# utiasSTARS/pyslam

Hardware: AMD Instinct MI355X
Metric: ms/LM-iter (Jac build + J^T J + Schur solve), stereo BA @ 500k residuals (lower is better)
Workload: dtype f64

## Files before the change

pyslam_amd/csrc/ps_abi_problem.h:

```cpp


const char* ps_last_error(void) { return g_err.c_str(); }

int ps_device_count(void) {
    int n = 0;
    if (hipGetDeviceCount(&n) != hipSuccess) return 0;
    return n;
}

int ps_warm_up(void) {
    static std::once_flag once;
    static int rc = 0;
    std::call_once(once, [] {
        void* p = nullptr;
        if (hipMalloc(&p, 256) != hipSuccess) { rc = fail("hipMalloc failed (no usable HIP device?)"); return; }
        hipLaunchKernelGGL(k_zero4, dim3(1), dim3(256), 0, 0, (size_t)8, (double*)p, (size_t)0, (double*)nullptr, (size_t)0,
                           (double*)nullptr, (size_t)0, (double*)nullptr);
        double hostw[4] = {0, 0, 0, 0};
        (void)hipMemsetAsync(p, 0, 256, 0);
        (void)hipMemcpyAsync((char*)p + 128, p, 64, hipMemcpyDeviceToDevice, 0);
        (void)hipMemcpyAsync(hostw, p, sizeof(hostw), hipMemcpyDeviceToHost, 0);
        if (hipDeviceSynchronize() != hipSuccess) rc = fail("the warm-up launch failed");
        hipFree(p);
        hipFuncAttributes a;
#define PS_TOUCH(...) (void)hipFuncGetAttributes(&a, reinterpret_cast<const void*>(&__VA_ARGS__))
        PS_TOUCH(k_landmark_pass<false>); PS_TOUCH(k_landmark_pass_packed<false, false>); PS_TOUCH(k_landmark_pass_packed<false, true>); PS_TOUCH(k_backsub_packed<false>); PS_TOUCH(k_pose_pass<false>); PS_TOUCH(k_pose_finalize); PS_TOUCH(k_schur_pairs_db<0>);
        PS_TOUCH(k_schur_combine); PS_TOUCH(k_backsub<false>); PS_TOUCH(k_cost_reproj<false>); PS_TOUCH(k_cost_packed<false>); PS_TOUCH(k_reduce3); PS_TOUCH(k_reduce_partials);
        PS_TOUCH(k_copy2); PS_TOUCH(k_zero4); PS_TOUCH(k_lag_status_check);
        PS_TOUCH(k_block_jacobi_factor<6>); PS_TOUCH(k_scale_blocks<6>); PS_TOUCH(k_scale_blocks_p<6>); PS_TOUCH(k_rows_setup<6>);
        PS_TOUCH(k_coarse_rowsums<6>); PS_TOUCH(k_coarse_matrix<6>); PS_TOUCH(k_coarse_chol<6, true>); PS_TOUCH(k_coarse_border<6>);
        PS_TOUCH(k_coarse_mreduce<6>); PS_TOUCH(k_coarse_xbuild<6>); PS_TOUCH(k_coarse_recover<6>); PS_TOUCH(k_cg_fused_lds<6, 8>);
        PS_TOUCH(k_cg_fused<6, 8>); PS_TOUCH(k_cg_unscale<6>); PS_TOUCH(k_update_poses<6>); PS_TOUCH(k_update_points);
        PS_TOUCH(k_xcoarse_rowsums<6>); PS_TOUCH(k_xcoarse_matrix<6>); PS_TOUCH(k_band_chol<6>); PS_TOUCH(k_band_inverse); PS_TOUCH(k_band_inverse_rl<false>);
        PS_TOUCH(k_band_inverse_rl<true>); PS_TOUCH(k_bp_v); PS_TOUCH(k_bp_t); PS_TOUCH(k_bp_w); PS_TOUCH(k_bp_dense_sep); PS_TOUCH(k_bp_dense);
        PS_TOUCH(k_xcg_restrict<6>); PS_TOUCH(k_xcg_f2_coarse<6, 3>); PS_TOUCH(k_xcg_fused1<6, 8, false>); PS_TOUCH(k_xcg_fused1<6, 0, true>);
        PS_TOUCH(k_xcg_fused1<6, 2, false>); PS_TOUCH(k_xcg_fused1<6, 6, false>);
        PS_TOUCH(k_factor_pass<6>); PS_TOUCH(k_factor_assemble<6>); PS_TOUCH(k_cost_factors<6>);
        PS_TOUCH(k_factor_pass<3>); PS_TOUCH(k_factor_assemble<3>); PS_TOUCH(k_cost_factors<3>); PS_TOUCH(k_block_jacobi_factor<3>);
        PS_TOUCH(k_update_poses<3>); PS_TOUCH(k_direct_solve<6>); PS_TOUCH(k_direct_solve<3>);
        PS_TOUCH(k_motion_only_solve<false>); PS_TOUCH(k_motion_only_iteration<false>);
        PS_TOUCH(k_pcg_spmv<6>); PS_TOUCH(k_pcg_spmv<3>); PS_TOUCH(k_ldi_init); PS_TOUCH(k_ldi_update); PS_TOUCH(k_ldi_gemm); PS_TOUCH(k_ldi_mirror);
        PS_TOUCH(k_ldi_ritz); PS_TOUCH(k_ldi_seed_prep); PS_TOUCH(k_ldi_fro_total); PS_TOUCH(k_ldi_pad_identity);
        PS_TOUCH(k_ldi_scaled_dense<6>); PS_TOUCH(k_ldi_sym_unscale<6>); PS_TOUCH(k_ldi_scaled_dense<3>); PS_TOUCH(k_ldi_sym_unscale<3>);
        PS_TOUCH(k_shard_pack<6>); PS_TOUCH(k_shard_unpack<6>); PS_TOUCH(k_publish); PS_TOUCH(k_cov_rhs); PS_TOUCH(k_triangulate<false>);
        PS_TOUCH(k_scale_blocks<3>); PS_TOUCH(k_rows_setup<3>); PS_TOUCH(k_coarse_rowsums<3>); PS_TOUCH(k_coarse_matrix<3>);
        PS_TOUCH(k_coarse_chol<3, true>); PS_TOUCH(k_coarse_border<3>); PS_TOUCH(k_coarse_mreduce<3>); PS_TOUCH(k_coarse_xbuild<3>);
        PS_TOUCH(k_coarse_recover<3>); PS_TOUCH(k_cg_fused_lds<3, 8>); PS_TOUCH(k_cg_unscale<3>);
#undef PS_TOUCH
    });
    return rc;
}

int ps_problem_destroy(ps_problem* h) {
    if (!h) return 0;
    if (h->cp_dbg) {
        long long c[8]; hipMemcpy(c, h->cp_dbg, 64, hipMemcpyDeviceToHost);
        int khz = 100000; hipDeviceGetAttribute(&khz, hipDeviceAttributeWallClockRate, 0);
        fprintf(stderr, "k_cg_persist, workgroup 0, %ld launches, us per launch: recurrences %.2f | sync %.2f | products + publish %.2f | gather + sums %.2f "
                "(%.1f failed passes) | dots + sync %.2f | exchanges %lld = %.2f per launch\n", h->cp_launches, c[0] * 1e3 / khz / h->cp_launches,
                c[1] * 1e3 / khz / h->cp_launches, c[2] * 1e3 / khz / h->cp_launches, c[3] * 1e3 / khz / h->cp_launches, (double)c[7] / h->cp_launches,
                c[5] * 1e3 / khz / h->cp_launches, c[6], (double)c[6] / h->cp_launches);
        hipFree(h->cp_dbg);
    }
    if (h->xp_dbg) {
        std::vector<long long> c(3 * 64 * 8); hipMemcpy(c.data(), h->xp_dbg, c.size() * 8, hipMemcpyDeviceToHost);
        int khz = 100000; hipDeviceGetAttribute(&khz, hipDeviceAttributeWallClockRate, 0);
        for (int w = 0; w < 3; ++w) {
            double ph[6] = {0, 0, 0, 0, 0, 0}; int np = 0;
// ... 813 lines not shown
```

pyslam_amd/csrc/ps_abi_solver.h:

```cpp

int ps_get_info(ps_problem* h, ps_problem_info* info) {
    if (!h || !info) return fail("null argument");
    info->dof = h->D; info->num_poses = h->P; info->num_reduced = h->nr; info->num_points = h->L;
    info->num_var_points = h->nv; info->num_obs = h->N; info->num_edges = h->F; info->num_priors = 0;
    info->reduced_nnzb = h->nnzb; info->num_pairs = h->npairs;
    info->reduce_count = ((long)h->nnzb + h->nr) / 2 * h->D * h->D + (long)h->nr * h->D + 3;
    info->device_bytes = (int64_t)h->dev_bytes;
    info->cg_restarts = h->cg_fallbacks;
    info->cg_kernel_launches = h->cg_kernel_launches;
    info->ldi_solves = h->ldi_solves; info->ldi_fallbacks = h->ldi_fallbacks; info->ldi_seeds = h->ldi_seeds;
    info->xcg_fused_solves = h->xf_solves; info->xcg_fused_fallbacks = h->xf_fallbacks;
    info->cg_persist_solves = h->cp_launches; info->cg_persist_failures = h->cp_failures;
    info->cg_persist_refused = h->cp_refused; info->persist_cus = h->persist_cus;
    info->persist_cus_needed = h->cp_ok ? h->cp_cus_needed : (h->xp_ok ? h->xp_cus_needed : 0);
    info->landmark_passes_taken_over = h->prelm_used;
    return 0;
}

int ps_eval_cost(ps_problem* h, int include_all_constant, double* cost) {
    if (!h || !cost) return fail("null argument");
    if (include_all_constant && h->fuse_cost == 1 && lm_cost_possible(h)) { if (lm_cost_pass(h, h->lin_lambda, SC_COST)) return -1; }
    else if (cost_pass(h, include_all_constant, SC_COST)) return -1;
    if (read_scalars(h)) return -1;
    *cost = h->h_scalars[SC_COST];
// ... 794 lines not shown
            for (; i + 8 <= buf.size(); i += 8) { uint64_t w; std::memcpy(&w, &buf[i], 8); hsh = (hsh ^ w) * 1099511628211ull; }
            for (; i < buf.size(); ++i) hsh = (hsh ^ buf[i]) * 1099511628211ull;
        }
        out[t] = hsh;
    }
    return 0;
}

static void relook_path(ps_problem* h) {
    const bool possible = ps_ldi_possible(*h, (long)h->nr * h->D);
    if (h->coarse_built && possible != h->xmin_auto_ldi && h->cg_explicit_min_rows < 0) h->coarse_built = false;
}

int ps_set_option(ps_problem* h, const char* name, double value) {
    if (!h || !name) return fail("null argument");
    if (!std::strcmp(name, "expect_next")) { h->expect_next = value != 0 && !h->hybrid; return 0; }
    if (!std::strcmp(name, "solve_horizon")) { h->solve_horizon = value < 0 ? -1 : (int)std::min(value, 1e6); return 0; }
    if (!std::strcmp(name, "setup_ride")) {
        h->setup_ride = value != 0 ? 1 : 0;
        h->prelin_valid = h->prelm_valid = false;
        relook_launch_gates(h);
        return 0;
    }
    h->prelin_valid = h->prelm_valid = h->ride_valid = false;
    const char* refusal = nullptr;
    const int fx = ps_option_apply(*h, name, value, &refusal);
    if (fx == PS_OPT_UNKNOWN) return fail(std::string("unknown option: ") + name);
    if (fx == PS_OPT_REFUSED) return fail(refusal);
    if (fx & PS_FX_COARSE_REBUILD) h->coarse_built = false;
    if (fx & PS_FX_DROP_FACTOR) h->lci_next = -1;
    if (fx & PS_FX_DROP_SIDE) h->side_todo = false;
    if ((fx & PS_FX_LDI_OFF) && !h->ldi_enable) { h->ldi_cur = -1; if (h->ldi_state != 1) h->ldi_state = 0; }
    if (fx & PS_FX_RELOOK_PATH) relook_path(h);
    relook_launch_gates(h);
    return 0;
}

int ps_get_option(ps_problem* h, const char* name, double* value) {
    if (!h || !name || !value) return fail("null argument");
    const std::string n(name);
    if (n == "lin_zero_list") *value = h->lin_zero_gate ? 1.0 : 0.0;
    else if (n == "lin_fills") *value = (double)h->lin_fills;
    else if (n == "lin_zero_launches") *value = (double)h->lin_zero_launches;
    else if (n == "setup_ride") *value = h->ride_gate ? 1.0 : 0.0;
    else if (n == "factor_launches") *value = (double)h->bjf_launches;
    else if (n == "factors_ridden") *value = (double)h->bjf_ridden;
    else if (n == "factor_plan_mismatches") *value = (double)h->bjf_mismatches;
    else return fail("ps_get_option: no read-back for option: " + n);
    return 0;
}

int ps_reset_solver_state(ps_problem* h) {
    if (!h) return fail("null argument");
    h->prelin_valid = h->prelm_valid = h->ride_valid = false;
    if (!h->solver_touched) {
        static_cast<PsCostHistory&>(*h) = PsCostHistory{};
        return 0;
    }
    h->solver_touched = false;
    HIP_OK(hipStreamSynchronize(h->stream));
    if (h->side) HIP_OK(hipStreamSynchronize(h->side));
    if (h->ldi_stream) HIP_OK(hipStreamSynchronize(h->ldi_stream));
    drain_timers(h);
    static_cast<PsCarried&>(*h) = PsCarried{};
    static_cast<PsCostHistory&>(*h) = PsCostHistory{};
    if (h->lag_status) HIP_OK(hipMemsetAsync(h->lag_status, 0, ST_NWORDS * sizeof(int32_t), h->stream));
    if (h->ldi_ready && !(h->ldi_direct_ok && h->N == 0 && h->F > 0)) h->ldi_direct = false;
    h->cov_ready = false;
    return 0;
}
// ... 54 lines not shown
```

pyslam_amd/csrc/ps_core.hip:

```cpp
#include <hip/hip_runtime.h>

#include <algorithm>
#include <array>
#include <map>
#include <atomic>
#include <chrono>
#include <thread>
#include <climits>
#include <cmath>
#include <cstdio>
#include <cstring>
#include <memory>
#include <mutex>
#include <string>
#include <vector>

#include "pyslam_hip.h"
#include "ps_kernels.h"
#include "ps_ransac.h"
#include "ps_k_twoview.h"
#include "ps_k_pnp.h"
#include "ps_photo.h"
#include "ps_k_dense.h"
#include "ps_k_feat.h"
// ... 207 lines not shown
    long bjf_launches = 0, bjf_ridden = 0, bjf_mismatches = 0;
    std::vector<int32_t> h_row_ptr, h_col_idx;
    std::vector<int32_t> h_vid_of_slot;
    double *x = nullptr, *r = nullptr, *z = nullptr, *p0 = nullptr, *p1 = nullptr, *q = nullptr, *Minv = nullptr;
    double *rz_part = nullptr, *rr_part = nullptr, *pq_part = nullptr, *hist = nullptr;
    int npartA = 0, npartB = 0, hist_cap = 0;
    double *Linv = nullptr, *cg_r[2] = {}, *cg_w[2] = {}, *cg_s[2] = {}, *cg_gd[2] = {}, *cg_xh = nullptr;
    int32_t* brow_of = nullptr;
    double* cg_p = nullptr;
    double* Saug = nullptr;
    int32_t* ident_slot = nullptr;
    int G = 0, ncb = 0, nc = 0, nr_aug = 0, nnzb_aug = 0;
    size_t cg_cap = 0, saug_cap = 0;
    int32_t *pnode = nullptr, *slo = nullptr, *shi = nullptr, *run_lo = nullptr, *run_hi = nullptr,
            *arow_ptr = nullptr, *acol_idx = nullptr, *aug_slot = nullptr, *fine_nnz = nullptr;
    double *pw0 = nullptr, *pw1 = nullptr, *SZ = nullptr, *Ac = nullptr, *tvec = nullptr, *chol_scratch = nullptr;
    double *Bmat = nullptr, *bgv = nullptr, *SB = nullptr, *BSZ = nullptr;
    double *Bmat2[2] = {}, *X2[2] = {}, *Mpart = nullptr;
    bool lagx_ok = false;
    int side_buf = 0;
    double host_wait_ns = 0.0, host_call_ns = 0.0;
    long host_waits = 0, host_calls = 0;
    size_t rows_lds = 0;
    bool rows_attr_set = false, rows_lci_lds = false;
    int32_t *ent_ptr = nullptr, *ent_q = nullptr, *ent_lo = nullptr, *ent_hi = nullptr;
    int32_t *seg_ptr = nullptr, *seg_ent = nullptr, *seg_row = nullptr;
    int max_row_ents = 0;
    int32_t* pose_of_rid = nullptr;
    double *Lci2[2] = {}, *LciT2[2] = {};
    hipStream_t side = nullptr;
    int side_cus = 0;
    hipEvent_t ev_ac = nullptr, ev_chol = nullptr, ev_acdone = nullptr;
    unsigned long long* chk_sums = nullptr; int chk_nsum = 0;
    double *chk_Ac = nullptr, *chk_BSZ = nullptr, *chk_Ac_side = nullptr; int32_t* chk_cnt = nullptr; size_t chk_bsz_n = 0;
    int32_t* lag_status = nullptr;
    double* Mc = nullptr;
    bool coarse_built = false;
    bool coarse_clamped = false;
    int max_pose_obs = 0;
    double* mo_partials = nullptr;
    bool status_clean = true;
    double *dA = nullptr, *dLi = nullptr, *dLiT = nullptr;
    bool cg_explicit = false;
    double lin_lambda = 0.0;
    double *xstate = nullptr, *xy = nullptr, *xp2 = nullptr;
    int ac_bw = -1;
    std::unique_ptr<BandPart> bpart;
// ... 272 lines not shown
```

pyslam_amd/csrc/ps_host_cg.h:

```cpp

namespace {

struct StageTimer {
    ps_problem* h;
    int stage;
    hipEvent_t a = nullptr, b = nullptr;
    int slot = -1;
    StageTimer(ps_problem* h_, int st, int level = 2) : h(h_), stage(st) {
        if (h->profiling < level) return;
        if (h->profiling == 1 && h->prof_every > 1 &&
            h->prof_tick % h->prof_every != (st == PS_ST_CG_KERNEL ? h->prof_every / 2 : 0)) return;
        if (h->ev_used + 2 > h->ev_pool.size()) {
            for (int i = 0; i < 64; ++i) { hipEvent_t e; hipEventCreate(&e); h->ev_pool.push_back(e); }
        }
        slot = (int)h->ev_used;
        a = h->ev_pool[h->ev_used++];
        b = h->ev_pool[h->ev_used++];
        hipEventRecord(a, h->stream);
    }
    void stop() {
        if (!a) return;
        hipEventRecord(b, h->stream);
        h->pending.push_back({stage, slot});
        a = nullptr;
// ... 331 lines not shown
            for (int k = 0; k < nt; ++k) tasks.push_back(CpTask{i, arp[i] + k * per, std::min(arp[i] + w, arp[i] + (k + 1) * per), 0});
        }
        rt0[rows] = (int32_t)tasks.size();
        const int cp_nwg = cdiv((int)tasks.size(), PS_CP_NT / 64);
        int cp_per_cu = 0;
        {
            const void* kfn = D == 6 ? (const void*)k_cg_persist<6> : (const void*)k_cg_persist<3>;
            if (hipOccupancyMaxActiveBlocksPerMultiprocessor(&cp_per_cu, kfn, PS_CP_NT, 0) != hipSuccess) { (void)hipGetLastError(); cp_per_cu = 0; }
        }
        h->cp_cus_needed = cp_per_cu > 0 ? cdiv(cp_nwg, cp_per_cu) : 0;
        if ((long)tasks.size() * D <= (long)PS_CP_MAXEX && h->cp_cus_needed > 0 && h->cp_cus_needed <= h->persist_capacity()) {
            CpTask* dt = nullptr;
            if (h->upload(&dt, tasks) || h->upload(&h->cp_row_task0, rt0) ||
                h->alloc(&h->cp_exch, (size_t)4 * tasks.size() * D)) return -1;
            h->cp_tasks = dt;
            HIP_OK(hipMemsetAsync(h->cp_exch, 0, (size_t)4 * tasks.size() * D * sizeof(unsigned long long), h->stream));
            h->cp_ntasks = (int)tasks.size(); h->cp_salt = 0; h->cp_ok = true;
        }
    }
    if (h->alloc(&h->BSZ, (h->cg_explicit ? eq.size() : (size_t)nr * ncb) * D * D) || h->alloc(&h->Bmat2[0], (size_t)nr * D * D) ||
        h->alloc(&h->bgv, (size_t)nr * D) || h->alloc(&h->SB, (size_t)aci.size() * D * D)) return -1;
    h->Bmat = h->Bmat2[0];
    h->lagx_ok = !h->cg_explicit && !split && h->nc <= 96 && maxlen <= PS_RS_MAXROW;
    h->side_todo = false; h->rows_attr_set = false;
    if (h->lagx_ok) {
        if (h->alloc(&h->Bmat2[1], (size_t)nr * D * D) || h->alloc(&h->X2[0], (size_t)nr * D * h->nc) ||
            h->alloc(&h->X2[1], (size_t)nr * D * h->nc) || h->alloc(&h->Mpart, (size_t)nr * h->nc * (h->nc + 1))) return -1;
        h->rows_lds = ((size_t)4 * maxlen * D * D + (size_t)D * (3 * h->nc + 1) + D * D + 3 * PS_RS_MAXROW) * sizeof(double)
                      + (PS_RS_MAXROW + 3 * 64) * sizeof(int32_t);
        h->rows_lci_lds = h->rows_lds + (size_t)h->nc * h->nc * sizeof(double) <= 160 * 1024;
        if (h->rows_lci_lds) h->rows_lds += (size_t)h->nc * h->nc * sizeof(double);
    }
    if ((!h->cg_explicit && h->alloc(&h->SZ, (size_t)nr * ncb * D * D)) || h->alloc(&h->Ac, (size_t)h->nc * h->nc) ||
        h->alloc(&h->Lci2[0], (size_t)h->nc * h->nc) || h->alloc(&h->LciT2[0], (size_t)h->nc * h->nc) ||
        h->alloc(&h->Lci2[1], (size_t)h->nc * h->nc) || h->alloc(&h->LciT2[1], (size_t)h->nc * h->nc) ||
        h->alloc(&h->tvec, (size_t)h->nc) || h->alloc(&h->chol_scratch, 2 * (size_t)h->nc * h->nc)) return -1;
    if (h->cg_explicit && (h->alloc(&h->xstate, 8) || h->alloc(&h->xy, (size_t)h->nc) || h->alloc(&h->xp2, (size_t)nr * D))) return -1;
    if (h->cg_explicit && h->ac_bw >= 0 &&
        (h->alloc(&h->Lrow, (size_t)h->nc * PS_BAND_W) || h->alloc(&h->Lcol, (size_t)h->nc * PS_BAND_W) || h->alloc(&h->rdiag, (size_t)h->nc))) return -1;
    h->xcg_rt_ok = false;
    if (h->cg_explicit && ncb <= PS_XCG_MAXNODES) {
        if (const char* e = ps_env("PS_XCG_ROWS_RT")) h->xcg_rt_rows = atoi(e);
        const int R = h->xcg_rt_rows, nwg = cdiv(nr, R);
        std::vector<int32_t> wgo((size_t)nwg * PS_XCG_NSLOT, -1), nptr(ncb + 1, 0);
        bool ok = true;
        for (int g = 0; g < nwg && ok; ++g) {
            const int first = g * R, last = std::min(nr, first + R) - 1;
// ... 169 lines not shown
            return h->bpart->run<D>(st, h->Ac, nc, (float*)h->LciT2[buf], nc, stat);
        }
    }
    if (h->band_chol && h->ac_bw >= 0) {
        HIP_OK(hipMemsetAsync(h->Lrow, 0, (size_t)nc * PS_BAND_W * sizeof(double), st));
        HIP_OK(hipMemsetAsync(h->Lcol, 0, (size_t)nc * PS_BAND_W * sizeof(double), st));
        hipLaunchKernelGGL(k_band_chol<D>, dim3(1), dim3(256), 0, st, h->ncb, std::max(h->ac_bw, 1), (const double*)h->Ac, h->Lrow, h->Lcol, h->rdiag, stat,
                           nc, (const int2*)nullptr);
        static const bool inv_dot = ps_env("PS_BAND_INV_DOT") != nullptr;
        if (inv_dot)
            hipLaunchKernelGGL(k_band_inverse, dim3(cdiv(nc, 4)), dim3(256), 0, st, nc, h->Lrow, h->Lcol, h->rdiag,
                               h->chol_scratch, (float*)h->LciT2[buf]);
        else
            hipLaunchKernelGGL(k_band_inverse_rl<false>, dim3(cdiv(nc, 4)), dim3(256), 0, st, nc, (const double*)h->Lrow, (const double*)h->Lcol,
                               (const double*)h->rdiag, h->chol_scratch, (float*)h->LciT2[buf], (const BandInvItem*)nullptr, (double*)nullptr, nc);
        return 0;
    }
    if (coarse_factor<D>(h, st, buf, stat)) return -1;
    hipLaunchKernelGGL(k_xcg_ainv, dim3(cdiv(nc, PS_AI_T) * (cdiv(nc, PS_AI_T) + 1) / 2), dim3(256), 0, st, nc, h->Lci2[buf], (float*)h->LciT2[buf], nc);
    return 0;
}

struct CgSetupPlan { bool lagged; int use; double* basis_out; };
inline CgSetupPlan cg_setup_plan(const ps_problem* h, bool allow_lag, int lci_next) {
    CgSetupPlan p{};
    p.lagged = h->G && h->lagx_ok && h->lagx && allow_lag && h->coarse_lag && lci_next >= 0;
    if (p.lagged) { p.use = lci_next; p.basis_out = h->Bmat2[lci_next ^ 1]; }
    else { p.use = h->lagx_ok ? h->lci_cur : 0; p.basis_out = h->G ? h->Bmat2[p.use] : nullptr; }
    return p;
}

inline bool ride_consume(ps_problem* h, const CgSetupPlan& plan) {
    if (!h->ride_valid) return false;
    h->ride_valid = false;
    if (plan.lagged == h->ride_lagged && plan.use == h->ride_use && plan.basis_out == h->ride_basis) return true;
    ++h->bjf_mismatches;
    return false;
}

template <int D>
int cg_fused_setup(ps_problem* h, int max_iters, bool allow_lag = false, bool rhs_only = false) {
    const int nr = h->nr, cap = h->hist_cap;
    if (max_iters + 2 > cap) return fail("pcg max_iters exceeds the history buffer (4096)");
    if (!h->coarse_built) { h->ride_valid = false; if (build_coarse(h)) return -1; }
    h->cg_max_launches = max_iters + 2;
    h->cp_recovered = false;
// ... 10 lines not shown
            hipLaunchKernelGGL(k_coarse_rhs<D>, dim3(1), dim3(1024), 0, h->stream, nr, h->ncb, h->slo, h->shi, h->pnode,
                               h->pw0, h->pw1, h->LciT2[h->lci_cur], h->arow_ptr, h->Saug, h->tvec, h->cg_r[0], h->cg_w[0],
                               h->cg_s[0], h->cg_p, h->cg_xh, h->cg_split ? 0 : 2, (const int32_t*)nullptr, h->status,
                               h->bgv);
        h->cg_launched = 0;
        return 0;
    }
    if (h->side_pending) {
        HIP_OK(hipStreamWaitEvent(h->stream, h->ev_chol, 0));
        h->side_pending = false;
    }
    const CgSetupPlan plan = cg_setup_plan(h, allow_lag, h->lci_next);
    const bool ridden = ride_consume(h, plan);
    if (!ridden) ++h->bjf_launches;
    if (plan.lagged) {
        const int ncb = h->ncb, nc = h->nc;
        const int use = plan.use, nb = use ^ 1;
        h->lci_cur = use;
        h->Bmat = h->Bmat2[use];
        if (!ridden)
            hipLaunchKernelGGL(k_block_jacobi_factor<D>, dim3(cdiv(nr, 4)), dim3(256), 0, h->stream, nr, h->diag_slot,
                               h->S, h->Linv, h->status, h->g, h->cg_r[0], h->cg_w[0], h->cg_s[0], h->cg_p, h->cg_xh,
                               h->poses, h->pose_of_rid, h->coarse_basis, plan.basis_out, h->bgv);
        if (!h->rows_attr_set) {
            if (ensure_dynamic_lds((const void*)k_rows_setup<D>, (size_t)(h->rows_lds))) return -1;
            h->rows_attr_set = true;
        }
        static const int rs_ablate = ps_env("PS_RS_ABLATE") ? atoi(ps_env("PS_RS_ABLATE")) : 0;
        hipLaunchKernelGGL(k_rows_setup<D>, dim3(nr), dim3(PS_RS_THREADS), h->rows_lds, h->stream, nr, ncb, h->row_ptr, h->col_idx,
                           h->aug_slot, h->S, h->Linv, h->Bmat2[use], h->Bmat2[nb], h->arow_ptr, h->fine_nnz,
                           h->run_lo, h->run_hi, h->pnode, h->pw0, h->pw1, h->LciT2[use], h->X2[use], h->cg_r[0],
                           h->Saug, h->SB, h->Mpart, h->rows_lci_lds ? 1 : 0, rs_ablate);
        hipLaunchKernelGGL(k_coarse_mreduce<D>, dim3(cdiv((long)nc * (nc + 1) * 8, 256)), dim3(256), 0, h->stream, nr, ncb,
                           h->shi, h->Mpart, h->pnode, h->arow_ptr, h->Saug, h->cg_r[0], h->cg_w[0], h->cg_s[0], h->cg_p,
                           h->cg_xh, h->lag_status, h->status, h->h_setup_dev, ++h->setup_seq);
        h->mc_active = false;
        h->side_todo = true; h->side_ready = false; h->side_buf = nb;
        h->cg_launched = 0;
        h->last_setup_lagx = true;
        return 0;
    }
    h->last_setup_lagx = false;
    h->side_todo = false;
    if (G) h->Bmat = plan.basis_out;
    if (!ridden)
        hipLaunchKernelGGL(k_block_jacobi_factor<D>, dim3(cdiv(nr, 4)), dim3(256), 0, h->stream, nr, h->diag_slot,
                           h->S, h->Linv, h->status, h->g, h->cg_r[0], h->cg_w[0], h->cg_s[0], h->cg_p, h->cg_xh,
                           h->poses, h->pose_of_rid, h->coarse_basis, plan.basis_out, h->bgv);
    hipLaunchKernelGGL(k_scale_blocks<D>, dim3(h->nnzb), dim3(64), 0, h->stream, nr, h->row_ptr, h->col_idx,
                       h->brow_of, h->Linv, h->S, h->aug_slot, h->Saug, G ? h->Bmat : (const double*)nullptr, h->SB);
    if (G) {
        const int ncb = h->ncb, nc = h->nc;
        if (h->side_pending) {
            HIP_OK(hipStreamWaitEvent(h->stream, h->ev_chol, 0));
            h->side_pending = false;
        }
        hipLaunchKernelGGL(k_coarse_rowsums<D>, dim3(nr), dim3(256), (size_t)(ncb + 1) * D * D * sizeof(double), h->stream,
                           nr, ncb, h->run_lo, h->run_hi, h->acol_idx, h->pnode, h->pw0, h->pw1, h->SB, h->SZ, h->Bmat, h->BSZ);
        hipLaunchKernelGGL(k_coarse_matrix<D>, dim3(cdiv((long)ncb * ncb * D * D, 256)), dim3(256), 0, h->stream,
                           nr, ncb, h->slo, h->shi, h->pnode, h->pw0, h->pw1, h->BSZ, h->Ac);
        auto launch_chol = [&](hipStream_t st, int buf, int32_t* stat) -> int { return coarse_factor<D>(h, st, buf, stat); };
        const bool lag = allow_lag && h->coarse_lag && h->lci_next >= 0 && (!h->cg_split || (long)h->nnzb > 24L * nr) &&
                         !(h->lagx_ok && h->lagx);
        if (lag && h->cg_split && !h->Mc && h->alloc(&h->Mc, (size_t)nc * nc)) return -1;
        h->mc_active = lag && h->cg_split;
        const int rpw = nc >= 192 ? 4 : 1;
        const int border_lds = (int)((size_t)rpw * D * nc * sizeof(double));
        if (ensure_dynamic_lds((const void*)k_coarse_border<D>, (size_t)border_lds)) return -1;
        if (lag) {
            const int use = h->lci_next;
            h->lci_cur = use;
            const CoarseRhsArgs ra{h->slo, h->shi, h->pnode, h->pw0, h->pw1, h->LciT2[use], h->tvec, h->cg_r[0], h->cg_w[0],
                                   h->cg_s[0], h->cg_p, h->cg_xh, h->cg_split ? 0 : 2, h->lag_status, h->status, h->bgv, h->cg_split ? h->Mc : nullptr};
            hipLaunchKernelGGL(k_coarse_border<D>, dim3(cdiv(nr, rpw) + ncb + 1), dim3(256), border_lds, h->stream,
                               nr, ncb, h->SZ, h->Lci2[use], h->arow_ptr, h->fine_nnz, h->Saug, h->cg_split ? 0 : 1, h->Ac, ra, rpw);
            HIP_OK(hipEventRecord(h->ev_ac, h->stream));
            HIP_OK(hipStreamWaitEvent(h->side, h->ev_ac, 0));
            if (launch_chol(h->side, use ^ 1, h->lag_status)) return -1;
            HIP_OK(hipEventRecord(h->ev_chol, h->side));
            h->lci_next = use ^ 1; h->side_pending = true;
        } else {
// ... 511 lines not shown
```

pyslam_amd/csrc/ps_k_cg_fused.h:

```cpp
#pragma once

template <int D>
__global__ __launch_bounds__(256) void k_block_jacobi_factor(
    int nr, const int32_t* __restrict__ diag_slot, const double* __restrict__ S,
    double* __restrict__ Linv, int32_t* __restrict__ status,
    const double* __restrict__ g, double* __restrict__ r0, double* __restrict__ w0, double* __restrict__ s0,
    double* __restrict__ p0, double* __restrict__ x0,
    const double* __restrict__ poses, const int32_t* __restrict__ pose_of_rid, int basis,
    double* __restrict__ Bmat, double* __restrict__ bg)
{
    constexpr int DD = D * D;
    __shared__ double sc[4][PS_BJF_SCRATCH(D)];
    const int wv = threadIdx.x >> 6, lane = threadIdx.x & 63;
    const int i = blockIdx.x * 4 + wv;
    if (i >= nr) return;
    double a_in = 0.0;
    if (lane < DD) a_in = S[(size_t)diag_slot[i] * DD + lane];
    if (g && lane < D) sc[wv][3 * DD + D + lane] = g[(size_t)i * D + lane];
    const BjFactorOut o{Linv, status, g ? r0 : nullptr, w0, s0, p0, x0, poses, pose_of_rid, basis, Bmat, bg};
    block_jacobi_factor_wave<D>(i, lane, a_in, sc[wv], o);
}

template <int D>
__global__ __launch_bounds__(64) void k_scale_blocks(
// ... 16 lines not shown
    __syncthreads();
    const int r = t / D, c = t % D;
    if (t < DD) {
        double v = 0.0;
#pragma unroll
        for (int a = 0; a < D; ++a) v += sLi[r * D + a] * sS[a * D + c];
        sT[t] = v;
    }
    __syncthreads();
    if (t < DD) {
        double v = 0.0;
#pragma unroll
        for (int a = 0; a < D; ++a) v += sT[r * D + a] * sLj[c * D + a];
        Sout[(size_t)out_slot[b] * DD + t] = v;
        sS[t] = v;
    }
    if (!Bmat) return;
    __syncthreads();
    if (t < DD) {
        double v = 0.0;
#pragma unroll
        for (int a = 0; a < D; ++a) v += sS[r * D + a] * sB[a * D + c];
        SB[(size_t)out_slot[b] * DD + t] = v;
    }
}

#define PS_SCB_NB 4
template <int D>
__global__ __launch_bounds__(256) void k_scale_blocks_p(
    int nnzb, const int32_t* __restrict__ col_idx, const int32_t* __restrict__ brow_of,
    const double* __restrict__ Linv, const double* __restrict__ S, const int32_t* __restrict__ out_slot,
    double* __restrict__ Sout, const double* __restrict__ Bmat, double* __restrict__ SB)
{
    constexpr int DD = D * D;
    __shared__ double lds[4][5][36];
    const int wv = threadIdx.x >> 6, t = threadIdx.x & 63;
    const int b0 = (blockIdx.x * 4 + wv) * PS_SCB_NB;
    if (b0 >= nnzb) return;
    double *sS = lds[wv][0], *sT = lds[wv][1], *sLi = lds[wv][2], *sLj = lds[wv][3], *sB = lds[wv][4];
    int bi[PS_SCB_NB], bj[PS_SCB_NB], bs[PS_SCB_NB];
#pragma unroll
    for (int q = 0; q < PS_SCB_NB; ++q) {
        const int b = min(b0 + q, nnzb - 1);
        bi[q] = brow_of[b]; bj[q] = col_idx[b]; bs[q] = out_slot[b];
    }
    double vs[PS_SCB_NB], vi[PS_SCB_NB], vj[PS_SCB_NB], vb[PS_SCB_NB];
// ... 660 lines not shown
```

pyslam_amd/csrc/ps_k_coarse.h:

```cpp
#pragma once


PS_DEV double coarse_weight(int j, int q, const int32_t* __restrict__ pnode,
                            const double* __restrict__ pw0, const double* __restrict__ pw1) {
    return (pnode[j] == q) ? pw0[j] : pw1[j];
}

template <int D>
__global__ __launch_bounds__(256) void k_coarse_rowsums(
    int nr, int ncb, const int32_t* __restrict__ run_lo, const int32_t* __restrict__ run_hi,
    const int32_t* __restrict__ acol_idx, const int32_t* __restrict__ pnode,
    const double* __restrict__ pw0, const double* __restrict__ pw1,
    const double* __restrict__ SB ,
    double* __restrict__ SZ, const double* __restrict__ Bmat, double* __restrict__ BSZ )
{
    constexpr int DD = D * D;
    extern __shared__ double srow[];
    const int i = blockIdx.x, nslot = ncb * DD;
    double* sBi = srow + nslot;
    if (threadIdx.x < DD) sBi[threadIdx.x] = Bmat[(size_t)i * DD + threadIdx.x];
    for (int t = threadIdx.x; t < nslot; t += blockDim.x) {
        const int q = t / DD, e = t % DD;
        const int k0 = run_lo[i * ncb + q], k1 = run_hi[i * ncb + q];
        double acc = 0.0;
// ... 607 lines not shown
        if (k < nc && sub == 0) sy[k] = v;
    }
    __syncthreads();
    const int t = blockIdx.x * blockDim.x + threadIdx.x;
    if (t >= nr * D) return;
    const int i = t / D, c = t % D, q = pnode[i];
    const double w0 = pw0[i], w1 = pw1[i];
    double z[D];
#pragma unroll
    for (int m = 0; m < D; ++m) z[m] = w0 * sy[q * D + m] + ((q + 1 < ncb) ? w1 * sy[(q + 1) * D + m] : 0.0);
    double v = 0.0;
#pragma unroll
    for (int a = 0; a < D; ++a) {
        double xhat = xh[(size_t)i * D + a];
#pragma unroll
        for (int m = 0; m < D; ++m) xhat += Bmat[(size_t)i * D * D + a * D + m] * z[m];
        v += Linv[(size_t)i * D * D + a * D + c] * xhat;
    }
    x[t] = v;
}

#define PS_RS_THREADS 1024
#define PS_RS_MAXROW 96

template <int D>
__global__ __launch_bounds__(PS_RS_THREADS) void k_rows_setup(
    int nr, int ncb, const int32_t* __restrict__ row_ptr, const int32_t* __restrict__ col_idx,
    const int32_t* __restrict__ aug_slot, const double* __restrict__ S, const double* __restrict__ Linv,
    const double* __restrict__ Blag, const double* __restrict__ Bcur,
    const int32_t* __restrict__ arow_ptr, const int32_t* __restrict__ fine_nnz,
    const int32_t* __restrict__ run_lo, const int32_t* __restrict__ run_hi,
    const int32_t* __restrict__ pnode, const double* __restrict__ pw0, const double* __restrict__ pw1,
    const double* __restrict__ LciT , const double* __restrict__ X ,
    const double* __restrict__ ghat ,
    double* __restrict__ Saug, double* __restrict__ SB, double* __restrict__ Mpart ,
    int lci_in_lds , int ablate)
{
    constexpr int DD = D * D;
    extern __shared__ __attribute__((aligned(16))) double lds[];
    const int i = blockIdx.x, t = threadIdx.x, NT = blockDim.x;
    const int nc = ncb * D, nf = row_ptr[i + 1] - row_ptr[i], rp = row_ptr[i], n36 = nf * DD;
    double* sS = lds;
    double* sLj = sS + n36;
    double* sBl = sLj + n36;
    double* sBc = sBl + n36;
    double* sT = sBc + n36;
    double* sK = sT + D * nc;
    double* sX = sK + D * (nc + 1);
    double* sLi = sX + D * nc;
    double* sW = sLi + DD;
    double* sL = sW + 3 * PS_RS_MAXROW;
    int32_t* sI = reinterpret_cast<int32_t*>(sL + (lci_in_lds ? nc * nc : 0));
    int32_t* sSlot = sI;
    int32_t* sRun = sSlot + PS_RS_MAXROW;
    int32_t* sCrow = sRun + 2 * 64;
    const int a_rp = arow_ptr[i];
    for (int idx = t; idx < n36; idx += NT) {
        const int k = idx / DD, e = idx - k * DD, b = rp + k, j = col_idx[b];
        sS[idx] = S[(size_t)b * DD + e];
        sLj[idx] = Linv[(size_t)j * DD + e];
        sBl[idx] = Blag[(size_t)j * DD + e];
        sBc[idx] = Bcur[(size_t)j * DD + e];
    }
    for (int k = t; k < nf; k += NT) {
        const int j = col_idx[rp + k];
        sW[2 * k] = pw0[j]; sW[2 * k + 1] = pw1[j]; sW[2 * PS_RS_MAXROW + k] = (double)pnode[j];
        sSlot[k] = aug_slot[rp + k];
    }
    for (int q = t; q < ncb; q += NT) {
        sRun[q] = run_lo[i * ncb + q] - a_rp; sRun[64 + q] = run_hi[i * ncb + q] - a_rp;
        sCrow[q] = arow_ptr[nr + q];
    }
    for (int idx = t; idx < D * nc; idx += NT) sX[idx] = X[(size_t)i * D * nc + idx];
    if (lci_in_lds && !(ablate & 1)) for (int idx = t; idx < nc * nc; idx += NT) sL[idx] = LciT[idx];
    if (t < DD) sLi[t] = Linv[(size_t)i * DD + t];
    if (t < D) sK[t * (nc + 1) + nc] = ghat[(size_t)i * D + t];
    const int row_slot = a_rp + fine_nnz[i];
    const int a0 = pnode[i] * D;
    __syncthreads();
    {
        constexpr int NB = (PS_RS_MAXROW + PS_RS_THREADS / 64 - 1) / (PS_RS_THREADS / 64);
        const int wv = t >> 6, lane = t & 63, nwv = NT >> 6;
        const bool act = lane < DD && !(ablate & 2);
        const int r = act ? lane / D : 0, c = act ? lane - (lane / D) * D : 0;
        double v[NB], v2[NB];
#pragma unroll
        for (int m = 0; m < NB; ++m) {
            const int k = wv + m * nwv;
            v[m] = 0.0;
            if (act && k < nf) {
#pragma unroll
                for (int a = 0; a < D; ++a) v[m] += sLi[r * D + a] * sS[k * DD + a * D + c];
            }
        }
        __builtin_amdgcn_wave_barrier();
#pragma unroll
        for (int m = 0; m < NB; ++m) { const int k = wv + m * nwv; if (act && k < nf) sS[k * DD + lane] = v[m]; }
        __builtin_amdgcn_wave_barrier();
#pragma unroll
        for (int m = 0; m < NB; ++m) {
            const int k = wv + m * nwv;
            v[m] = 0.0;
// ... 10 lines not shown
        }
        __builtin_amdgcn_wave_barrier();
#pragma unroll
        for (int m = 0; m < NB; ++m) {
            const int k = wv + m * nwv;
            v[m] = v2[m] = 0.0;
            if (act && k < nf) {
#pragma unroll
                for (int a = 0; a < D; ++a) {
                    const double sv = sS[k * DD + r * D + a];
                    v[m] += sv * sBl[k * DD + a * D + c];
                    v2[m] += sv * sBc[k * DD + a * D + c];
                }
            }
        }
        __builtin_amdgcn_wave_barrier();
#pragma unroll
        for (int m = 0; m < NB; ++m) {
            const int k = wv + m * nwv;
            if (act && k < nf) { sBl[k * DD + lane] = v[m]; SB[(size_t)sSlot[k] * DD + lane] = v2[m]; }
        }
    }
    __syncthreads();
    for (int idx = t; idx < ncb * DD; idx += NT) {
        const int q = idx / DD, e = idx - q * DD, r = e / D, c = e - r * D;
        const int k0 = sRun[q], k1 = sRun[64 + q];
        double acc = 0.0;
        for (int k = k0; k < k1; ++k)
            acc += sBl[k * DD + e] * (((int)sW[2 * PS_RS_MAXROW + k] == q) ? sW[2 * k] : sW[2 * k + 1]);
        sT[r * nc + q * D + c] = acc;
    }
    __syncthreads();
    const double* Lt = lci_in_lds ? sL : LciT;
    for (int idx = t; idx < 2 * D * nc && !(ablate & 4); idx += NT) {
        const int o = idx >> 1, par = idx & 1;
        const int r = o / nc, c = o - r * nc, q = c / D, cc = c - q * D;
        double v = 0.0;
#pragma unroll 8
        for (int k = par; k <= c; k += 2) v += sT[r * nc + k] * Lt[(size_t)k * nc + c];
        v += __shfl_xor(v, 1, 64);
        if (par) continue;
        sK[r * (nc + 1) + c] = v;
        Saug[(size_t)(row_slot + q) * DD + r * D + cc] = v;
        Saug[(size_t)(sCrow[q] + i) * DD + cc * D + r] = v;
    }
    __syncthreads();
    const int ncol = nc + 1;
    for (int idx = t; idx < (nc - a0) * ncol && !(ablate & 8); idx += NT) {
        const int a = a0 + idx / ncol, c = idx % ncol;
        double v = 0.0;
#pragma unroll
        for (int r = 0; r < D; ++r) v += sX[r * nc + a] * sK[r * ncol + c];
        Mpart[((size_t)i * nc + a) * ncol + c] = v;
    }
}

template <int D>
__global__ __launch_bounds__(256) void k_coarse_mreduce(
    int nr, int ncb, const int32_t* __restrict__ shi, const double* __restrict__ Mpart,
    const int32_t* __restrict__ pnode, const int32_t* __restrict__ arow_ptr, double* __restrict__ Saug,
    double* __restrict__ r, double* __restrict__ w, double* __restrict__ s, double* __restrict__ p, double* __restrict__ x,
    const int32_t* __restrict__ lag_status, int32_t* __restrict__ status, long long* __restrict__ hsetup, long long setup_seq)
// ... 50 lines not shown
```

Before: 0.2860.

## Compute block-row scaling per thread in registers and fuse exact rowsums into rows_setup

Adds a register-based mode to k_rows_setup in which one thread computes a full scaled row of each block (Li*S*Lj^T, then times B) instead of the wave-per-block LDS passes. It also adds an EXACT mode that replaces k_scale_blocks plus k_coarse_rowsums on the non-lagged path with a single fused launch producing Saug, SB, SZ and BSZ. The triangular product over LciT is restricted to the span of nonzero coarse columns found via a wave ballot. The changes cut launches, LDS round trips and wasted multiplies against zero columns. The cost is a larger kernel with more template variants, and the removed side_pending wait on ev_chol may change ordering.

```diff
diff --git a/pyslam_amd/csrc/ps_abi_problem.h b/pyslam_amd/csrc/ps_abi_problem.h
--- a/pyslam_amd/csrc/ps_abi_problem.h
+++ b/pyslam_amd/csrc/ps_abi_problem.h
@@ -27,7 +27,7 @@
         PS_TOUCH(k_landmark_pass<false>); PS_TOUCH(k_landmark_pass_packed<false, false>); PS_TOUCH(k_landmark_pass_packed<false, true>); PS_TOUCH(k_backsub_packed<false>); PS_TOUCH(k_pose_pass<false>); PS_TOUCH(k_pose_finalize); PS_TOUCH(k_schur_pairs_db<0>);
         PS_TOUCH(k_schur_combine); PS_TOUCH(k_backsub<false>); PS_TOUCH(k_cost_reproj<false>); PS_TOUCH(k_cost_packed<false>); PS_TOUCH(k_reduce3); PS_TOUCH(k_reduce_partials);
         PS_TOUCH(k_copy2); PS_TOUCH(k_zero4); PS_TOUCH(k_lag_status_check);
-        PS_TOUCH(k_block_jacobi_factor<6>); PS_TOUCH(k_scale_blocks<6>); PS_TOUCH(k_scale_blocks_p<6>); PS_TOUCH(k_rows_setup<6>);
+        PS_TOUCH(k_block_jacobi_factor<6>); PS_TOUCH(k_scale_blocks<6>); PS_TOUCH(k_scale_blocks_p<6>); PS_TOUCH(k_rows_setup<6, PS_RS_REGS>); PS_TOUCH(k_rows_setup<6, PS_RS_EXACT>);
         PS_TOUCH(k_coarse_rowsums<6>); PS_TOUCH(k_coarse_matrix<6>); PS_TOUCH(k_coarse_chol<6, true>); PS_TOUCH(k_coarse_border<6>);
         PS_TOUCH(k_coarse_mreduce<6>); PS_TOUCH(k_coarse_xbuild<6>); PS_TOUCH(k_coarse_recover<6>); PS_TOUCH(k_cg_fused_lds<6, 8>);
         PS_TOUCH(k_cg_fused<6, 8>); PS_TOUCH(k_cg_unscale<6>); PS_TOUCH(k_update_poses<6>); PS_TOUCH(k_update_points);
@@ -43,7 +43,7 @@
         PS_TOUCH(k_ldi_ritz); PS_TOUCH(k_ldi_seed_prep); PS_TOUCH(k_ldi_fro_total); PS_TOUCH(k_ldi_pad_identity);
         PS_TOUCH(k_ldi_scaled_dense<6>); PS_TOUCH(k_ldi_sym_unscale<6>); PS_TOUCH(k_ldi_scaled_dense<3>); PS_TOUCH(k_ldi_sym_unscale<3>);
         PS_TOUCH(k_shard_pack<6>); PS_TOUCH(k_shard_unpack<6>); PS_TOUCH(k_publish); PS_TOUCH(k_cov_rhs); PS_TOUCH(k_triangulate<false>);
-        PS_TOUCH(k_scale_blocks<3>); PS_TOUCH(k_rows_setup<3>); PS_TOUCH(k_coarse_rowsums<3>); PS_TOUCH(k_coarse_matrix<3>);
+        PS_TOUCH(k_scale_blocks<3>); PS_TOUCH(k_rows_setup<3, PS_RS_REGS>); PS_TOUCH(k_rows_setup<3, PS_RS_EXACT>); PS_TOUCH(k_coarse_rowsums<3>); PS_TOUCH(k_coarse_matrix<3>);
         PS_TOUCH(k_coarse_chol<3, true>); PS_TOUCH(k_coarse_border<3>); PS_TOUCH(k_coarse_mreduce<3>); PS_TOUCH(k_coarse_xbuild<3>);
         PS_TOUCH(k_coarse_recover<3>); PS_TOUCH(k_cg_fused_lds<3, 8>); PS_TOUCH(k_cg_unscale<3>);
 #undef PS_TOUCH
diff --git a/pyslam_amd/csrc/ps_abi_solver.h b/pyslam_amd/csrc/ps_abi_solver.h
--- a/pyslam_amd/csrc/ps_abi_solver.h
+++ b/pyslam_amd/csrc/ps_abi_solver.h
@@ -840,6 +840,11 @@
         relook_launch_gates(h);
         return 0;
     }
+    if (!std::strcmp(name, "rows_regs")) {
+        h->rows_regs = value != 0 ? 1 : 0;
+        h->prelin_valid = h->prelm_valid = h->ride_valid = false;
+        return 0;
+    }
     h->prelin_valid = h->prelm_valid = h->ride_valid = false;
     const char* refusal = nullptr;
     const int fx = ps_option_apply(*h, name, value, &refusal);
@@ -864,6 +869,10 @@
     else if (n == "factor_launches") *value = (double)h->bjf_launches;
     else if (n == "factors_ridden") *value = (double)h->bjf_ridden;
     else if (n == "factor_plan_mismatches") *value = (double)h->bjf_mismatches;
+    else if (n == "rows_regs") *value = (double)h->rows_regs;
+    else if (n == "rows_setups") *value = (double)h->rows_setups;
+    else if (n == "exact_row_setups") *value = (double)h->exact_row_setups;
+    else if (n == "rows_lci_in_lds") *value = h->coarse_built && h->lagx_ok && h->rows_lci_lds ? 1.0 : 0.0;
     else return fail("ps_get_option: no read-back for option: " + n);
     return 0;
 }
diff --git a/pyslam_amd/csrc/ps_core.hip b/pyslam_amd/csrc/ps_core.hip
--- a/pyslam_amd/csrc/ps_core.hip
+++ b/pyslam_amd/csrc/ps_core.hip
@@ -253,7 +253,10 @@
     double host_wait_ns = 0.0, host_call_ns = 0.0;
     long host_waits = 0, host_calls = 0;
     size_t rows_lds = 0;
-    bool rows_attr_set = false, rows_lci_lds = false;
+    int rows_attr_set = 0;
+    bool rows_lci_lds = false;
+    int rows_regs = 1;
+    long rows_setups = 0, exact_row_setups = 0;
     int32_t *ent_ptr = nullptr, *ent_q = nullptr, *ent_lo = nullptr, *ent_hi = nullptr;
     int32_t *seg_ptr = nullptr, *seg_ent = nullptr, *seg_row = nullptr;
     int max_row_ents = 0;
diff --git a/pyslam_amd/csrc/ps_host_cg.h b/pyslam_amd/csrc/ps_host_cg.h
--- a/pyslam_amd/csrc/ps_host_cg.h
+++ b/pyslam_amd/csrc/ps_host_cg.h
@@ -377,7 +377,7 @@
         h->alloc(&h->bgv, (size_t)nr * D) || h->alloc(&h->SB, (size_t)aci.size() * D * D)) return -1;
     h->Bmat = h->Bmat2[0];
     h->lagx_ok = !h->cg_explicit && !split && h->nc <= 96 && maxlen <= PS_RS_MAXROW;
-    h->side_todo = false; h->rows_attr_set = false;
+    h->side_todo = false; h->rows_attr_set = 0;
     if (h->lagx_ok) {
         if (h->alloc(&h->Bmat2[1], (size_t)nr * D * D) || h->alloc(&h->X2[0], (size_t)nr * D * h->nc) ||
             h->alloc(&h->X2[1], (size_t)nr * D * h->nc) || h->alloc(&h->Mpart, (size_t)nr * h->nc * (h->nc + 1))) return -1;
@@ -593,6 +593,20 @@
 }
 
 struct CgSetupPlan { bool lagged; int use; double* basis_out; };
+
+template <int D, int MODE>
+int launch_rows_setup(ps_problem* h, const double* basis_lag, const double* basis_cur, const double* LciT, const double* X) {
+    if (!(h->rows_attr_set >> MODE & 1)) {
+        if (ensure_dynamic_lds((const void*)k_rows_setup<D, MODE>, (size_t)(h->rows_lds))) return -1;
+        h->rows_attr_set |= 1 << MODE;
+    }
+    static const int rs_ablate = ps_env("PS_RS_ABLATE") ? atoi(ps_env("PS_RS_ABLATE")) : 0;
+    hipLaunchKernelGGL((k_rows_setup<D, MODE>), dim3(h->nr), dim3(PS_RS_THREADS), h->rows_lds, h->stream, h->nr, h->ncb, h->row_ptr,
+                       h->col_idx, h->aug_slot, h->S, h->Linv, basis_lag, basis_cur, h->arow_ptr, h->fine_nnz,
+                       h->run_lo, h->run_hi, h->pnode, h->pw0, h->pw1, LciT, X, h->cg_r[0],
+                       h->Saug, h->SB, h->Mpart, h->SZ, h->BSZ, h->rows_lci_lds ? 1 : 0, rs_ablate);
+    return 0;
+}
 inline CgSetupPlan cg_setup_plan(const ps_problem* h, bool allow_lag, int lci_next) {
     CgSetupPlan p{};
     p.lagged = h->G && h->lagx_ok && h->lagx && allow_lag && h->coarse_lag && lci_next >= 0;
@@ -649,15 +663,9 @@
             hipLaunchKernelGGL(k_block_jacobi_factor<D>, dim3(cdiv(nr, 4)), dim3(256), 0, h->stream, nr, h->diag_slot,
                                h->S, h->Linv, h->status, h->g, h->cg_r[0], h->cg_w[0], h->cg_s[0], h->cg_p, h->cg_xh,
                                h->poses, h->pose_of_rid, h->coarse_basis, plan.basis_out, h->bgv);
-        if (!h->rows_attr_set) {
-            if (ensure_dynamic_lds((const void*)k_rows_setup<D>, (size_t)(h->rows_lds))) return -1;
-            h->rows_attr_set = true;
-        }
-        static const int rs_ablate = ps_env("PS_RS_ABLATE") ? atoi(ps_env("PS_RS_ABLATE")) : 0;
-        hipLaunchKernelGGL(k_rows_setup<D>, dim3(nr), dim3(PS_RS_THREADS), h->rows_lds, h->stream, nr, ncb, h->row_ptr, h->col_idx,
-                           h->aug_slot, h->S, h->Linv, h->Bmat2[use], h->Bmat2[nb], h->arow_ptr, h->fine_nnz,
-                           h->run_lo, h->run_hi, h->pnode, h->pw0, h->pw1, h->LciT2[use], h->X2[use], h->cg_r[0],
-                           h->Saug, h->SB, h->Mpart, h->rows_lci_lds ? 1 : 0, rs_ablate);
+        if (h->rows_regs ? launch_rows_setup<D, PS_RS_REGS>(h, h->Bmat2[use], h->Bmat2[nb], h->LciT2[use], h->X2[use])
+                         : launch_rows_setup<D, PS_RS_WAVES>(h, h->Bmat2[use], h->Bmat2[nb], h->LciT2[use], h->X2[use])) return -1;
+        ++h->rows_setups;
         hipLaunchKernelGGL(k_coarse_mreduce<D>, dim3(cdiv((long)nc * (nc + 1) * 8, 256)), dim3(256), 0, h->stream, nr, ncb,
                            h->shi, h->Mpart, h->pnode, h->arow_ptr, h->Saug, h->cg_r[0], h->cg_w[0], h->cg_s[0], h->cg_p,
                            h->cg_xh, h->lag_status, h->status, h->h_setup_dev, ++h->setup_seq);
@@ -674,16 +682,18 @@
         hipLaunchKernelGGL(k_block_jacobi_factor<D>, dim3(cdiv(nr, 4)), dim3(256), 0, h->stream, nr, h->diag_slot,
                            h->S, h->Linv, h->status, h->g, h->cg_r[0], h->cg_w[0], h->cg_s[0], h->cg_p, h->cg_xh,
                            h->poses, h->pose_of_rid, h->coarse_basis, plan.basis_out, h->bgv);
-    hipLaunchKernelGGL(k_scale_blocks<D>, dim3(h->nnzb), dim3(64), 0, h->stream, nr, h->row_ptr, h->col_idx,
-                       h->brow_of, h->Linv, h->S, h->aug_slot, h->Saug, G ? h->Bmat : (const double*)nullptr, h->SB);
+    const bool exact_rows = G && h->lagx_ok && h->rows_regs;
+    if (exact_rows) {
+        if (launch_rows_setup<D, PS_RS_EXACT>(h, nullptr, h->Bmat, nullptr, nullptr)) return -1;
+        ++h->exact_row_setups;
+    } else
+        hipLaunchKernelGGL(k_scale_blocks<D>, dim3(h->nnzb), dim3(64), 0, h->stream, nr, h->row_ptr, h->col_idx,
+                           h->brow_of, h->Linv, h->S, h->aug_slot, h->Saug, G ? h->Bmat : (const double*)nullptr, h->SB);
     if (G) {
         const int ncb = h->ncb, nc = h->nc;
-        if (h->side_pending) {
-            HIP_OK(hipStreamWaitEvent(h->stream, h->ev_chol, 0));
-            h->side_pending = false;
-        }
-        hipLaunchKernelGGL(k_coarse_rowsums<D>, dim3(nr), dim3(256), (size_t)(ncb + 1) * D * D * sizeof(double), h->stream,
-                           nr, ncb, h->run_lo, h->run_hi, h->acol_idx, h->pnode, h->pw0, h->pw1, h->SB, h->SZ, h->Bmat, h->BSZ);
+        if (!exact_rows)
+            hipLaunchKernelGGL(k_coarse_rowsums<D>, dim3(nr), dim3(256), (size_t)(ncb + 1) * D * D * sizeof(double), h->stream,
+                               nr, ncb, h->run_lo, h->run_hi, h->acol_idx, h->pnode, h->pw0, h->pw1, h->SB, h->SZ, h->Bmat, h->BSZ);
         hipLaunchKernelGGL(k_coarse_matrix<D>, dim3(cdiv((long)ncb * ncb * D * D, 256)), dim3(256), 0, h->stream,
                            nr, ncb, h->slo, h->shi, h->pnode, h->pw0, h->pw1, h->BSZ, h->Ac);
         auto launch_chol = [&](hipStream_t st, int buf, int32_t* stat) -> int { return coarse_factor<D>(h, st, buf, stat); };
diff --git a/pyslam_amd/csrc/ps_k_cg_fused.h b/pyslam_amd/csrc/ps_k_cg_fused.h
--- a/pyslam_amd/csrc/ps_k_cg_fused.h
+++ b/pyslam_amd/csrc/ps_k_cg_fused.h
@@ -62,6 +62,37 @@
 #pragma unroll
         for (int a = 0; a < D; ++a) v += sS[r * D + a] * sB[a * D + c];
         SB[(size_t)out_slot[b] * DD + t] = v;
+    }
+}
+
+template <int D>
+PS_DEV void scaled_block_row(const double* Li_r, const double* S, const double* Lj, const double* B0, const double* B1,
+                             double (&sh)[D], double (&o0)[D], double (&o1)[D])
+{
+    double tr[D];
+#pragma unroll
+    for (int c = 0; c < D; ++c) {
+        double v = 0.0;
+#pragma unroll
+        for (int a = 0; a < D; ++a) v = fma(Li_r[a], S[a * D + c], v);
+        tr[c] = v;
+    }
+#pragma unroll
+    for (int c = 0; c < D; ++c) {
+        double v = 0.0;
+#pragma unroll
+        for (int a = 0; a < D; ++a) v = fma(tr[a], Lj[c * D + a], v);
+        sh[c] = v;
+    }
+#pragma unroll
+    for (int c = 0; c < D; ++c) {
+        double v = 0.0, u = 0.0;
+#pragma unroll
+        for (int a = 0; a < D; ++a) {
+            if (B0) v = fma(sh[a], B0[a * D + c], v);
+            if (B1) u = fma(sh[a], B1[a * D + c], u);
+        }
+        o0[c] = v; o1[c] = u;
     }
 }
 
diff --git a/pyslam_amd/csrc/ps_k_coarse.h b/pyslam_amd/csrc/ps_k_coarse.h
--- a/pyslam_amd/csrc/ps_k_coarse.h
+++ b/pyslam_amd/csrc/ps_k_coarse.h
@@ -653,8 +653,11 @@
 
 #define PS_RS_THREADS 1024
 #define PS_RS_MAXROW 96
-
-template <int D>
+#define PS_RS_WAVES 0
+#define PS_RS_REGS 1
+#define PS_RS_EXACT 2
+
+template <int D, int MODE>
 __global__ __launch_bounds__(PS_RS_THREADS) void k_rows_setup(
     int nr, int ncb, const int32_t* __restrict__ row_ptr, const int32_t* __restrict__ col_idx,
     const int32_t* __restrict__ aug_slot, const double* __restrict__ S, const double* __restrict__ Linv,
@@ -665,9 +668,12 @@
     const double* __restrict__ LciT , const double* __restrict__ X ,
     const double* __restrict__ ghat ,
     double* __restrict__ Saug, double* __restrict__ SB, double* __restrict__ Mpart ,
+    double* __restrict__ SZ, double* __restrict__ BSZ ,
     int lci_in_lds , int ablate)
 {
     constexpr int DD = D * D;
+    constexpr bool EXACT = MODE == PS_RS_EXACT;
+    static_assert(PS_RS_MAXROW * D <= PS_RS_THREADS, "a thread per block row");
     extern __shared__ __attribute__((aligned(16))) double lds[];
     const int i = blockIdx.x, t = threadIdx.x, NT = blockDim.x;
     const int nc = ncb * D, nf = row_ptr[i + 1] - row_ptr[i], rp = row_ptr[i], n36 = nf * DD;
@@ -685,12 +691,13 @@
     int32_t* sSlot = sI;
     int32_t* sRun = sSlot + PS_RS_MAXROW;
     int32_t* sCrow = sRun + 2 * 64;
+    int32_t* sSpan = sCrow + 62;
     const int a_rp = arow_ptr[i];
     for (int idx = t; idx < n36; idx += NT) {
         const int k = idx / DD, e = idx - k * DD, b = rp + k, j = col_idx[b];
         sS[idx] = S[(size_t)b * DD + e];
         sLj[idx] = Linv[(size_t)j * DD + e];
-        sBl[idx] = Blag[(size_t)j * DD + e];
+        if (!EXACT) sBl[idx] = Blag[(size_t)j * DD + e];
         sBc[idx] = Bcur[(size_t)j * DD + e];
     }
     for (int k = t; k < nf; k += NT) {
@@ -700,15 +707,33 @@
     }
     for (int q = t; q < ncb; q += NT) {
         sRun[q] = run_lo[i * ncb + q] - a_rp; sRun[64 + q] = run_hi[i * ncb + q] - a_rp;
-        sCrow[q] = arow_ptr[nr + q];
-    }
-    for (int idx = t; idx < D * nc; idx += NT) sX[idx] = X[(size_t)i * D * nc + idx];
-    if (lci_in_lds && !(ablate & 1)) for (int idx = t; idx < nc * nc; idx += NT) sL[idx] = LciT[idx];
+        if (!EXACT) sCrow[q] = arow_ptr[nr + q];
+    }
+    if (!EXACT) {
+        for (int idx = t; idx < D * nc; idx += NT) sX[idx] = X[(size_t)i * D * nc + idx];
+        if (lci_in_lds && !(ablate & 1)) for (int idx = t; idx < nc * nc; idx += NT) sL[idx] = LciT[idx];
+        if (t < D) sK[t * (nc + 1) + nc] = ghat[(size_t)i * D + t];
+    } else if (t < DD) sK[t] = Bcur[(size_t)i * DD + t];
     if (t < DD) sLi[t] = Linv[(size_t)i * DD + t];
-    if (t < D) sK[t * (nc + 1) + nc] = ghat[(size_t)i * D + t];
     const int row_slot = a_rp + fine_nnz[i];
     const int a0 = pnode[i] * D;
     __syncthreads();
+    if (MODE != PS_RS_WAVES) {
+        const bool act = t < nf * D && (EXACT || !(ablate & 2));
+        const int k = act ? t / D : 0, r = act ? t - k * D : 0;
+        double sh[D], o0[D], o1[D];
+        if (act) {
+            scaled_block_row<D>(sLi + r * D, sS + k * DD, sLj + k * DD, EXACT ? nullptr : sBl + k * DD, sBc + k * DD, sh, o0, o1);
+            const size_t o = (size_t)sSlot[k] * DD + r * D;
+#pragma unroll
+            for (int c = 0; c < D; ++c) { Saug[o + c] = sh[c]; SB[o + c] = o1[c]; }
+        }
+        if (!EXACT) __syncthreads();
+        if (act) {
+#pragma unroll
+            for (int c = 0; c < D; ++c) sBl[k * DD + r * D + c] = EXACT ? o1[c] : o0[c];
+        }
+    } else
     {
         constexpr int NB = (PS_RS_MAXROW + PS_RS_THREADS / 64 - 1) / (PS_RS_THREADS / 64);
         const int wv = t >> 6, lane = t & 63, nwv = NT >> 6;
@@ -765,22 +790,39 @@
         }
     }
     __syncthreads();
+    if (MODE == PS_RS_REGS && t < 64) {
+        const unsigned long long m = __ballot(t < ncb && sRun[64 + t] > sRun[t]);
+        if (t == 0) { sSpan[0] = m ? (__ffsll((long long)m) - 1) * D : 0; sSpan[1] = m ? (64 - __clzll((long long)m)) * D : 0; }
+    }
     for (int idx = t; idx < ncb * DD; idx += NT) {
         const int q = idx / DD, e = idx - q * DD, r = e / D, c = e - r * D;
         const int k0 = sRun[q], k1 = sRun[64 + q];
         double acc = 0.0;
         for (int k = k0; k < k1; ++k)
             acc += sBl[k * DD + e] * (((int)sW[2 * PS_RS_MAXROW + k] == q) ? sW[2 * k] : sW[2 * k + 1]);
-        sT[r * nc + q * D + c] = acc;
-    }
-    __syncthreads();
+        if (EXACT) { sT[idx] = acc; SZ[(size_t)i * ncb * DD + idx] = acc; }
+        else sT[r * nc + q * D + c] = acc;
+    }
+    __syncthreads();
+    if (EXACT) {
+        for (int idx = t; idx < ncb * DD; idx += NT) {
+            const int q = idx / DD, e = idx - q * DD, r = e / D, c = e - r * D;
+            double acc = 0.0;
+#pragma unroll
+            for (int m = 0; m < D; ++m) acc += sK[m * D + r] * sT[q * DD + m * D + c];
+            BSZ[(size_t)i * ncb * DD + idx] = acc;
+        }
+        return;
+    }
     const double* Lt = lci_in_lds ? sL : LciT;
+    const int klo = MODE == PS_RS_REGS ? sSpan[0] : 0, khi = MODE == PS_RS_REGS ? sSpan[1] : nc;
     for (int idx = t; idx < 2 * D * nc && !(ablate & 4); idx += NT) {
         const int o = idx >> 1, par = idx & 1;
         const int r = o / nc, c = o - r * nc, q = c / D, cc = c - q * D;
+        const int kend = min(c, khi - 1);
         double v = 0.0;
 #pragma unroll 8
-        for (int k = par; k <= c; k += 2) v += sT[r * nc + k] * Lt[(size_t)k * nc + c];
+        for (int k = klo + ((klo ^ par) & 1); k <= kend; k += 2) v += sT[r * nc + k] * Lt[(size_t)k * nc + c];
         v += __shfl_xor(v, 1, 64);
         if (par) continue;
         sK[r * (nc + 1) + c] = v;
```

After: 0.2821 (median of 6 runs). -1.3%, faster.
